# laiviet/ed-gated-gcn

Measured on AMD Instinct MI355X. Metric: gated_gcn_forward_edges_per_sec, higher is better.
Workload: dtype f32 (fp16 MFMA + block-scaled fp8 correction MFMA, fp32 accumulate)

## Files before the change

### ed-gated-gcn_amd/csrc/f16mx8_core.h

```cpp
#pragma once
#include "bf16x3_core.h"
#include "lab_hooks.h"

namespace ggcn {
namespace mx8 {

using namespace bx3;

typedef _Float16 f16x8 __attribute__((ext_vector_type(8)));
typedef int i32x8 __attribute__((ext_vector_type(8)));
typedef int i32x4 __attribute__((ext_vector_type(4)));

#ifndef GGCN_WH8_STORED
#define GGCN_WH8_STORED 0
#endif
constexpr int kWh8Bytes = GGCN_WH8_STORED ? 64 * 16 : 0;
constexpr int kOffWl8 = 2 * 1024, kOffWh8 = kOffWl8 + 64 * 16, kOffScales = kOffWh8 + kWh8Bytes;
constexpr int STAGE_PACK_BYTES = kOffScales + 64 * 4;
constexpr int XL_SHIFT = 11;
constexpr int SCALE_XL = 127 - XL_SHIFT, SCALE_XH = 127;

static __device__ unsigned int g_range_flag;
constexpr float kWindow = 448.0f;
constexpr float kHalfMax = 65504.0f;
__device__ __forceinline__ void range_verdict(float amax, float hb_scale = 0.0f, float hb_add = 0.0f, bool window = true)
{
    unsigned bits = 0u;
    if (window && amax > kWindow) bits |= 2u;
    if (amax >= kHalfMax) bits |= 1u;
    if (amax * hb_scale + hb_add >= kHalfMax) bits |= 4u;
    if (bits) atomicOr(&g_range_flag, bits);
}
#define GGCN_RANGE_FLAG_TU(fn)                                                                          \
    namespace {                                                                                         \
    __global__ void fn##_kernel(unsigned int *dst, int clear)                                           \
    {                                                                                                   \
        const unsigned int v = mx8::g_range_flag;                                                       \
        if (v) atomicOr(dst, v);                                                                        \
        if (clear) mx8::g_range_flag = 0u;                                                              \
    }                                                                                                   \
    }                                                                                                   \
    int fn(unsigned int *dst, int clear, hipStream_t st)                                                \
    {                                                                                                   \
        hipLaunchKernelGGL(fn##_kernel, dim3(1), dim3(1), 0, st, dst, clear);                           \
        return check_launch("ggcn_range_flag");                                                         \
    }
constexpr int PACK_TRAILER_BYTES = 16;
__device__ __forceinline__ float amax3(float x0, float x1, float m)
{
    float d;
    asm("v_max3_f32 %0, |%1|, |%2|, %3" : "=v"(d) : "v"(x0), "v"(x1), "v"(m));
    return d;
}

struct Split4 {
    uint32_t h01, h23;
    int l8, h8;
};
__device__ __forceinline__ int undef_vgpr() { int r; asm volatile("" : "=v"(r)); return r; }
__device__ __forceinline__ Split4 split4(float x0, float x1, float x2, float x3, float &amax)
{
    typedef _Float16 h2 __attribute__((ext_vector_type(2)));
    typedef float f2 __attribute__((ext_vector_type(2)));
    typedef short s2 __attribute__((ext_vector_type(2)));
    const h2 p0 = __builtin_convertvector(f2{x0, x1}, h2);
    const h2 p1 = __builtin_convertvector(f2{x2, x3}, h2);
    float r0, r1, r2, r3;
    asm("v_fma_mix_f32 %0, %1, -1.0, %2 op_sel_hi:[1,0,0]" : "=v"(r0) : "v"(p0), "v"(x0));
    asm("v_fma_mix_f32 %0, %1, -1.0, %2 op_sel:[1,0,0] op_sel_hi:[1,0,0]" : "=v"(r1) : "v"(p0), "v"(x1));
    asm("v_fma_mix_f32 %0, %1, -1.0, %2 op_sel_hi:[1,0,0]" : "=v"(r2) : "v"(p1), "v"(x2));
    asm("v_fma_mix_f32 %0, %1, -1.0, %2 op_sel:[1,0,0] op_sel_hi:[1,0,0]" : "=v"(r3) : "v"(p1), "v"(x3));
    constexpr float inv = 1.0f / (float)(1 << XL_SHIFT);
    s2 q = __builtin_bit_cast(s2, undef_vgpr());
    q = __builtin_amdgcn_cvt_scalef32_pk_fp8_f32(q, r0, r1, inv, false);
    q = __builtin_amdgcn_cvt_scalef32_pk_fp8_f32(q, r2, r3, inv, true);
    amax = amax3(x2, x3, amax3(x0, x1, amax));
    int h8 = __builtin_amdgcn_cvt_pk_fp8_f32(x0, x1, undef_vgpr(), false);
    h8 = __builtin_amdgcn_cvt_pk_fp8_f32(x2, x3, h8, true);
    Split4 o;
    o.h01 = __builtin_bit_cast(uint32_t, p0);
    o.h23 = __builtin_bit_cast(uint32_t, p1);
    o.l8 = __builtin_bit_cast(int, q);
    o.h8 = h8;
    return o;
}

__device__ __forceinline__ void set_cvt_saturate(bool on) { __builtin_amdgcn_s_setreg(1 | (23 << 6), on ? 1 : 0); }

__device__ __forceinline__ int q_lds_off(int row, int chunk)
{
    return row * ROWB + ((chunk ^ ((row >> 2) & 3) ^ (((row >> 1) & 1) << 1)) << 4);
}

#define GGCN_SB() __builtin_amdgcn_sched_barrier(0)
#define GGCN_ON(bit) constexpr (!((GGCN_LAB_OFF) & (bit)))

template <typename AT>
struct BufX {
    const AT *base;
    uint32_t bytes;
    uint32_t off[Geom<AT>::NP];
};
template <typename AT>
__device__ __forceinline__ BufX<AT> make_bufx(const AT *X, int64_t ldx, int64_t base_row, int64_t total_rows,
                                              const int (&rel)[Geom<AT>::NP], int tid)
{
    BufX<AT> b;
    const int64_t left = (total_rows - base_row) * ldx * (int64_t)sizeof(AT);
    b.base = X + base_row * ldx;
    b.bytes = (uint32_t)(left < 0x7fffffff ? left : 0x7fffffff);
#pragma unroll
    for (int i = 0; i < Geom<AT>::NP; ++i)
        b.off[i] = rel[i] < 0 ? 0x80000000u
                              : (uint32_t)(((int64_t)rel[i] * ldx + (tid % Geom<AT>::TPR) * Geom<AT>::EPT) * (int64_t)sizeof(AT));
    return b;
}
#ifndef GGCN_LAB_W2
#define GGCN_LAB_W2 0
#endif
template <typename AT, bool AVEC, bool KFULL, bool ZROWS, bool RBLK = false, bool BUF = false, int NB = 4, bool XS = false, int XP = 4, int SLOT0 = 0>
__device__ __forceinline__ void mainloop(const AT *const (&arow)[Geom<AT>::NP], const bool (&avalid)[Geom<AT>::NP],
                                         const char *__restrict__ wpack, int K, int stages_packed, int wm,
                                         int nt0, int n_tiles_total, char *lds, f32x16 (&acc)[4][RN], int rot = 0, int nblk = 4,
                                         float *amax_out = nullptr, const BufX<AT> *bufx = nullptr, float xscale = 1.0f, int pass0 = 0)
{
    static_assert(!BUF || (AVEC && KFULL && sizeof(AT) == 4), "buffer loads: whole 16-byte pieces of fp32 rows");
    static_assert(NB >= 1 && NB <= 4 && (NB == 4 || (sizeof(AT) == 4 && !RBLK)), "NB < 4: fp32 rows (pass i = block i), no run-time count");
    constexpr int NPL0 = Geom<AT>::NP < NB ? Geom<AT>::NP : NB;
    constexpr int NPL = NPL0 < XP ? NPL0 : XP;
    static_assert(XP == 4 || (sizeof(AT) == 4 && NB == 4 && !RBLK), "XP < 4: fp32 rows, whole tiles");
    static_assert(SLOT0 >= 0 && SLOT0 + XP <= 4, "the staging passes sit behind the stage's four row-block slots");
    using G = Geom<AT>;
    constexpr int EPT = G::EPT, NP = G::NP, NQ = EPT / 4;
    static_assert(BK == 32 && NP <= 4 && RN == 2, "the slot schedule below is written for BK = 32, <= 4 passes, RN = 2");
    const int tid = threadIdx.x & (kThreads - 1);
    const int lane = tid & 63;
    const int s_k = (tid % G::TPR) * EPT;

    set_cvt_saturate(true);
    float amax = 0.0f;

    constexpr int kRsrcFlags = 0x00020000;
    __amdgpu_buffer_rsrc_t xr, wr;
    if constexpr (BUF) {
        xr = __builtin_amdgcn_make_buffer_rsrc(const_cast<AT *>(bufx->base), 0, (int)bufx->bytes, kRsrcFlags);
        wr = __builtin_amdgcn_make_buffer_rsrc(const_cast<char *>(wpack), 0, 0x7fffffff, kRsrcFlags);
    }
    float ra[NP][EPT];
    auto load_a_pass = [&](int i, int k0) {
        const int gk = k0 + s_k;
        if constexpr (BUF) {
            const float4 t = __builtin_bit_cast(float4, __builtin_amdgcn_raw_buffer_load_b128(xr, bufx->off[i], k0 * (int)sizeof(AT), 0));
            ra[i][0] = t.x; ra[i][1] = t.y; ra[i][2] = t.z; ra[i][3] = t.w;
        } else if constexpr (AVEC) {
            load16<AT>(arow[i] + ((KFULL || gk < K) ? gk : 0), ra[i]);
        } else {
#pragma unroll
            for (int c = 0; c < EPT; ++c) ra[i][c] = elem_to_float(arow[i][(gk + c < K) ? gk + c : 0]);
        }
    };
    Split4 sp[NQ];
    auto split_pass = [&](int i, int k0) {
        const int gk = k0 + s_k;
#pragma unroll
        for (int q = 0; q < NQ; ++q) {
            float x[4];
#pragma unroll
            for (int c = 0; c < 4; ++c) {
                x[c] = ra[i][4 * q + c];
                if constexpr (!KFULL || ZROWS) {
                    bool in = true;
                    if constexpr (!KFULL) in = gk + 4 * q + c < K;
                    if constexpr (ZROWS && !BUF) in = in && avalid[i];
                    x[c] = in ? x[c] : 0.0f;
                }
                if constexpr (XS) x[c] *= xscale;
            }
            sp[q] = split4(x[0], x[1], x[2], x[3], amax);
        }
    };
    auto write_pass = [&](int buf, int i) {
        char *h_plane = lds + buf * (2 * BM * ROWB);
        char *q_plane = h_plane + BM * ROWB;
        const int row = stage_row<AT>(XP == 4 ? i : i + pass0);
#pragma unroll
        for (int q = 0; q < NQ; ++q) {
            const int kq = s_k + 4 * q;
            *reinterpret_cast<uint2 *>(h_plane + a_lds_off(row, kq >> 3) + (kq & 4) * 2) = make_uint2(sp[q].h01, sp[q].h23);
            const int g = kq >> 2, hh = (g >> 1) & 1, pos = (g & 1) + 2 * (g >> 2);
            *reinterpret_cast<uint32_t *>(q_plane + q_lds_off(row, hh) + 4 * pos) = (uint32_t)sp[q].l8;
            *reinterpret_cast<uint32_t *>(q_plane + q_lds_off(row, 2 + hh) + 4 * pos) = (uint32_t)sp[q].h8;
        }
    };

    const char *bbase[RN];
#pragma unroll
    for (int j = 0; j < RN; ++j) {
        const int ntc = nt0 + j < n_tiles_total ? nt0 + j : n_tiles_total - 1;
        bbase[j] = wpack + (int64_t)ntc * stages_packed * STAGE_PACK_BYTES + lane * 16;
    }
    uint32_t wtile[RN];
#pragma unroll
    for (int j = 0; j < RN; ++j) {
        const int ntc = nt0 + j < n_tiles_total ? nt0 + j : n_tiles_total - 1;
        wtile[j] = (uint32_t)ntc * (uint32_t)stages_packed * STAGE_PACK_BYTES;
    }
    const uint32_t lane16 = lane * 16, lane4 = lane * 4;
    auto load_bf = [&](int st, f16x8 (&b0)[RN], f16x8 (&b1)[RN]) {
        st = st < stages_packed ? st : stages_packed - 1;
#pragma unroll
        for (int j = 0; j < RN; ++j) {
            if constexpr (BUF) {
                const uint32_t so = wtile[j] + (uint32_t)st * STAGE_PACK_BYTES;
                b0[j] = __builtin_bit_cast(f16x8, __builtin_amdgcn_raw_buffer_load_b128(wr, lane16, so, 0));
                b1[j] = __builtin_bit_cast(f16x8, __builtin_amdgcn_raw_buffer_load_b128(wr, lane16, so + 1024, 0));
            } else {
                const char *p = bbase[j] + (int64_t)st * STAGE_PACK_BYTES;
                b0[j] = *reinterpret_cast<const f16x8 *>(p);
                b1[j] = *reinterpret_cast<const f16x8 *>(p + 1024);
            }
        }
    };
    auto load_bq = [&](int st, i32x4 (&b)[RN], int (&sc)[RN]) {
        st = st < stages_packed ? st : stages_packed - 1;
#pragma unroll
        for (int j = 0; j < RN; ++j) {
            if constexpr (BUF) {
                const uint32_t so = wtile[j] + (uint32_t)st * STAGE_PACK_BYTES;
                b[j] = __builtin_bit_cast(i32x4, __builtin_amdgcn_raw_buffer_load_b128(wr, lane16, so + kOffWl8, 0));
                sc[j] = __builtin_amdgcn_raw_buffer_load_b32(wr, lane4, so + kOffScales, 0);
            } else {
                const char *p = bbase[j] + (int64_t)st * STAGE_PACK_BYTES;
                b[j] = *reinterpret_cast<const i32x4 *>(p + kOffWl8);
                sc[j] = *reinterpret_cast<const int *>(p + kOffScales - lane * 12);
            }
        }
    };
    auto load_wh8 = [&](int st, i32x4 (&b)[RN]) {
        st = st < stages_packed ? st : stages_packed - 1;
#pragma unroll
        for (int j = 0; j < RN; ++j) {
            if constexpr (BUF) b[j] = __builtin_bit_cast(i32x4, __builtin_amdgcn_raw_buffer_load_b128(wr, lane16, wtile[j] + (uint32_t)st * STAGE_PACK_BYTES + kOffWh8, 0));
            else b[j] = *reinterpret_cast<const i32x4 *>(bbase[j] + (int64_t)st * STAGE_PACK_BYTES + kOffWh8);
        }
    };
    auto wh8_of = [&](const f16x8 &f0, const f16x8 &f1, int sc) -> i32x4 {
        typedef _Float16 h2 __attribute__((ext_vector_type(2)));
        typedef short s2 __attribute__((ext_vector_type(2)));
        const float inv = __builtin_bit_cast(float, (sc & 0xff00) << 15);
        i32x4 o;
#pragma unroll
        for (int d = 0; d < 4; ++d) {
            const f16x8 &f = d < 2 ? f0 : f1;
            const int e = (d & 1) * 4;
            s2 q = __builtin_bit_cast(s2, undef_vgpr());
            q = __builtin_amdgcn_cvt_scalef32_pk_fp8_f16(q, h2{f[e], f[e + 1]}, inv, false);
            q = __builtin_amdgcn_cvt_scalef32_pk_fp8_f16(q, h2{f[e + 2], f[e + 3]}, inv, true);
            o[d] = __builtin_bit_cast(int, q);
        }
        return o;
    };

    const int f_row = wm * 128 + (lane & 31);
    const int f_half = lane >> 5;
    const int scale_a = f_half ? SCALE_XH : SCALE_XL;
    auto read_h = [&](int buf, int i, f16x8 (&a)[2]) {
        const char *h_plane = lds + buf * (2 * BM * ROWB);
        const int row = f_row + i * 32;
        a[0] = *reinterpret_cast<const f16x8 *>(h_plane + a_lds_off(row, f_half));
        a[1] = *reinterpret_cast<const f16x8 *>(h_plane + a_lds_off(row, 2 + f_half));
    };
    auto read_q = [&](int buf, int i, i32x8 &a) {
        const char *q_plane = lds + buf * (2 * BM * ROWB) + BM * ROWB;
        const int row = f_row + i * 32;
        const i32x4 lo = *reinterpret_cast<const i32x4 *>(q_plane + q_lds_off(row, f_half));
        const i32x4 hi = *reinterpret_cast<const i32x4 *>(q_plane + q_lds_off(row, 2 + f_half));
        a = __builtin_shufflevector(lo, hi, 0, 1, 2, 3, 4, 5, 6, 7);
    };

#pragma unroll
    for (int i = 0; i < 4; ++i)
#pragma unroll
        for (int j = 0; j < RN; ++j)
#pragma unroll
            for (int r = 0; r < 16; ++r) acc[i][j][r] = 0.0f;

    constexpr bool W2 = (GGCN_LAB_W2) != 0;
    f16x8 bset0[W2 ? 2 : 1][RN], bset1[W2 ? 2 : 1][RN];
    f16x8 (&b0)[RN] = bset0[0], (&b1)[RN] = bset1[0];
    i32x4 bq[RN];
    i32x4 bw[RN];
    int sq[RN];
    const int stages = (K + BK - 1) / BK;

    auto kstage = [&](int n) {
        n = n < stages ? n : stages - 1;
        const int s = n + rot;
        return s >= stages ? s - stages : s;
    };
#pragma unroll
    for (int p = 0; p < NPL; ++p) load_a_pass(p, kstage(0) * BK);
    load_bf(kstage(0), b0, b1);
#pragma unroll
    for (int p = 0; p < NPL; ++p) {
        split_pass(p, kstage(0) * BK);
        write_pass(0, p);
    }
#pragma unroll
    for (int p = 0; p < NPL; ++p) load_a_pass(p, kstage(1) * BK);
    __syncthreads();

    f16x8 lab_h[2];
    i32x8 lab_q;
    i32x8 lab_bm[RN];
    if constexpr ((GGCN_LAB_OFF) != 0) {
        read_h(0, 0, lab_h);
        read_q(0, 0, lab_q);
        load_bq(kstage(0), bq, sq);
        if constexpr (GGCN_WH8_STORED) load_wh8(kstage(0), bw);
#pragma unroll
        for (int j = 0; j < RN; ++j) {
            const i32x4 w = GGCN_WH8_STORED ? bw[j] : wh8_of(b0[j], b1[j], sq[j]);
            lab_bm[j] = i32x8{w[0], w[1], w[2], w[3], bq[j][0], bq[j][1], bq[j][2], bq[j][3]};
        }
    }
    auto stage = [&](int st, auto bufc) {
        constexpr int buf = decltype(bufc)::value;
        const int k_next1 = kstage(st + 1) * BK;
        const int ka = kstage(st + 2) * BK;
        f16x8 ah[2][2];
        i32x8 aq[2];
        if GGCN_ON(8) read_h(buf, 0, ah[0]); else { ah[0][0] = lab_h[0]; ah[0][1] = lab_h[1]; }
        if GGCN_ON(16) { load_bq(kstage(st), bq, sq); if constexpr (GGCN_WH8_STORED) load_wh8(kstage(st), bw); }
        f16x8 (&b0)[RN] = bset0[W2 ? buf : 0], (&b1)[RN] = bset1[W2 ? buf : 0];
        if constexpr (W2) { if GGCN_ON(16) load_bf(kstage(st + 1), bset0[buf ^ 1], bset1[buf ^ 1]); }
        GGCN_SB();
#pragma unroll
        for (int i = 0; i < NB; ++i) {
            if GGCN_ON(8) {
                if (i < NB - 1) read_h(buf, i + 1, ah[(i + 1) & 1]);
                else read_q(buf, 0, aq[0]);
            } else {
                if (i < NB - 1) { ah[(i + 1) & 1][0] = lab_h[0]; ah[(i + 1) & 1][1] = lab_h[1]; }
                else aq[0] = lab_q;
            }
            GGCN_SB();
            if (!RBLK || i < nblk) acc[i][0] = __builtin_amdgcn_mfma_f32_32x32x16_f16(ah[i & 1][0], b0[0], acc[i][0], 0, 0, 0);
            GGCN_SB();
            if GGCN_ON(2) { if (i - SLOT0 >= 0 && i - SLOT0 < NP && i - SLOT0 < GGCN_LAB_XPASSES && i - SLOT0 < XP) split_pass(i - SLOT0, k_next1); }
            GGCN_SB();
            if (!RBLK || i < nblk) acc[i][1] = __builtin_amdgcn_mfma_f32_32x32x16_f16(ah[i & 1][0], b0[1], acc[i][1], 0, 0, 0);
            GGCN_SB();
            if GGCN_ON(4) { if (i - SLOT0 >= 0 && i - SLOT0 < NP && i - SLOT0 < GGCN_LAB_XPASSES && i - SLOT0 < XP) write_pass(buf ^ 1, i - SLOT0); }
            else { _Pragma("unroll") for (int q = 0; q < NQ; ++q) asm volatile("" :: "v"(sp[q].h01), "v"(sp[q].h23), "v"(sp[q].l8), "v"(sp[q].h8)); }
            GGCN_SB();
            if (!RBLK || i < nblk) acc[i][0] = __builtin_amdgcn_mfma_f32_32x32x16_f16(ah[i & 1][1], b1[0], acc[i][0], 0, 0, 0);
            GGCN_SB();
            if GGCN_ON(1) { if (i - SLOT0 >= 0 && i - SLOT0 < NP && i - SLOT0 < GGCN_LAB_XPASSES && i - SLOT0 < XP) load_a_pass(i - SLOT0, ka); }
            else { if (i < NP) { _Pragma("unroll") for (int c = 0; c < EPT; ++c) asm volatile("" : "+v"(ra[i][c])); } }
            GGCN_SB();
            if (!RBLK || i < nblk) acc[i][1] = __builtin_amdgcn_mfma_f32_32x32x16_f16(ah[i & 1][1], b1[1], acc[i][1], 0, 0, 0);
            GGCN_SB();
        }
        i32x8 bm[RN];
        auto make_bm = [&](int j) {
            if GGCN_ON(32) {
                i32x4 w;
                if constexpr (GGCN_WH8_STORED) w = bw[j];
                else w = wh8_of(b0[j], b1[j], sq[j]);
                bm[j] = i32x8{w[0], w[1], w[2], w[3], bq[j][0], bq[j][1], bq[j][2], bq[j][3]};
            } else {
                bm[j] = lab_bm[j];
            }
        };
        make_bm(0);
        if constexpr (!(GGCN_LAB_WH8)) make_bm(1);
        GGCN_SB();
#pragma unroll
        for (int i = 0; i < NB; ++i) {
            if GGCN_ON(8) { if (i < NB - 1) read_q(buf, i + 1, aq[(i + 1) & 1]); }
            else { if (i < NB - 1) aq[(i + 1) & 1] = lab_q; }
            GGCN_SB();
            if (!RBLK || i < nblk) acc[i][0] = __builtin_amdgcn_mfma_scale_f32_32x32x64_f8f6f4(aq[i & 1], bm[0], acc[i][0], GGCN_LAB_MXFMT, GGCN_LAB_MXFMT, 0, scale_a, 0, sq[0]);
            GGCN_SB();
            if constexpr (GGCN_LAB_WH8) { if (i == 0) make_bm(1); }
            if constexpr (!W2) { if GGCN_ON(16) { if (i == 0) load_bf(kstage(st + 1), b0, b1); } }
            GGCN_SB();
            if (!RBLK || i < nblk) acc[i][1] = __builtin_amdgcn_mfma_scale_f32_32x32x64_f8f6f4(aq[i & 1], bm[1], acc[i][1], GGCN_LAB_MXFMT, GGCN_LAB_MXFMT, 0, scale_a, 0, sq[1]);
            GGCN_SB();
        }
        if GGCN_ON(64) __syncthreads();
    };
    int st = 0;
    for (; st + 1 < stages; st += 2) {
        stage(st, std::integral_constant<int, 0>{});
        stage(st + 1, std::integral_constant<int, 1>{});
    }
    if (st < stages) stage(st, std::integral_constant<int, 0>{});
    set_cvt_saturate(false);
    if (amax_out) *amax_out = amax;
    else range_verdict(amax);
}
#undef GGCN_SB
#undef GGCN_ON

}
}
```

### ed-gated-gcn_amd/csrc/fused_block8.hip

```cpp
#include "fused_common.h"

#include <cstdlib>

namespace ggcn {
namespace {

constexpr int kB8Threads = 512;
constexpr int kB8Lds = kLdsBytes + 2 * kEpiLdsBytes;

__device__ __forceinline__ bool getenv_slot_same(const FusedArgs &a) { return (a.k_steps & 0x20000000) != 0; }

template <int BASE>
__device__ __forceinline__ float staged_mid_max(const char *lds, bool dma, int lane)
{
    if (dma) {
        const float4 m4 = *reinterpret_cast<const float4 *>(lds + EpiLds<BASE>::kBias + BN * 4 + lane * 16);
        float mm = fmaxf(fmaxf(fabsf(m4.x), fabsf(m4.y)), fmaxf(fabsf(m4.z), fabsf(m4.w)));
#pragma unroll
        for (int d = 32; d >= 1; d >>= 1) mm = fmaxf(mm, __shfl_xor(mm, d));
        return mm;
    }
    const float4 mm = *reinterpret_cast<const float4 *>(lds + EpiLds<BASE>::kMidMax);
    return fmaxf(fmaxf(mm.x, mm.y), fmaxf(mm.z, mm.w));
}

template <bool FULLT, bool VST>
__global__ __launch_bounds__(kB8Threads, 1) void block_fused8_kernel(const FusedArgs a)
{
    extern __shared__ __attribute__((aligned(16))) char lds[];
    const int B = a.B, T = a.T, K = a.K, F = a.F;
    int n_wgi, g_tile;
    if (a.n_parts == 2) {
        const int xcd = blockIdx.x & 7, qb = blockIdx.x >> 3;
        const int total = a.g_tiles * a.n_wg, per_xcd = (total + 7) >> 3;
        const int w = xcd * per_xcd + qb;
        if (qb >= per_xcd || w >= total) return;
        n_wgi = w / a.g_tiles;
        g_tile = w - n_wgi * a.g_tiles;
    } else {
        if (!tile_of_block(blockIdx.x, a.g_tiles, a.n_wg, g_tile, n_wgi)) return;
    }

    const int tid8 = threadIdx.x;
    const unsigned long long t_start = a.stamps ? __builtin_amdgcn_s_memrealtime() : 0;
    const int group = __builtin_amdgcn_readfirstlane(tid8 >> 8);
    const int tid = tid8 & 255;
    const int wave = __builtin_amdgcn_readfirstlane(tid >> 6);
    const LayerPart &lp = a.part[group];
    const int gt0 = g_tile * 4, g0 = gt0;
    const int n_tiles_total = (F + NT - 1) / NT;
    const int nt0 = n_wgi * (BN / NT) + wave * RN;

    constexpr int NP = Geom<float>::NP;
    const float *arow[NP];
    bool avalid[NP];
    int rel[NP];
#pragma unroll
    for (int i = 0; i < NP; ++i) {
        const int row = stage_row<float>(i < 2 ? i + 2 * group : 0);
        const int g = gt0 + (row >> 5), r = row & 31;
        avalid[i] = i < 2 && (g < B) && (FULLT || r < T);
        arow[i] = a.X;
        rel[i] = avalid[i] ? (row >> 5) * T + (row & 31) : -1;
    }
    const bool dma = (a.n_wg * BN == F) && (gt0 + 4 <= B) && a.ov_in == nullptr && a.ov_out == nullptr && (a.k_steps & 0x40000000) != 0;
    const int k_steps = a.k_steps & 0x1fffffff;
    if (dma) {
        if (group == 0) stage_epilogue_operands_dma<kLdsBytes>(a, lp, g0, n_wgi, lds, tid);
        else stage_epilogue_operands_dma<kLdsBytes + kEpiLdsBytes>(a, lp, g0, n_wgi, lds, tid);
    } else {
        if (group == 0) stage_epilogue_operands<kLdsBytes>(a, lp, g0, n_wgi, lds, tid);
        else stage_epilogue_operands<kLdsBytes + kEpiLdsBytes>(a, lp, g0, n_wgi, lds, tid);
    }

    f32x16 acc[4][RN];
    float amax;
    const int64_t pack_bytes = (int64_t)n_tiles_total * (k_steps / 2) * mx8::STAGE_PACK_BYTES;
    const float bw1 = *reinterpret_cast<const float *>(a.part[0].wpack + pack_bytes);
    const float bw12 = *reinterpret_cast<const float *>(a.part[1].wpack + pack_bytes);
    const unsigned long long t_loop0 = a.stamps ? __builtin_amdgcn_s_memrealtime() : 0;
    mx8::BufX<float> bx = mx8::make_bufx<float>(a.X, a.ldx, (int64_t)gt0 * T, (int64_t)B * T, rel, tid);
    if (group == 0 || getenv_slot_same(a))
        mx8::mainloop<float, true, true, !FULLT, false, true, 4, false, 2, 0>(arow, avalid, lp.wpack, K, k_steps / 2, 0, nt0, n_tiles_total, lds, acc, 0, 4,
                                                                               &amax, &bx, 1.0f, 2 * group);
    else
        mx8::mainloop<float, true, true, !FULLT, false, true, 4, false, 2, 2>(arow, avalid, lp.wpack, K, k_steps / 2, 0, nt0, n_tiles_total, lds, acc, 0, 4,
                                                                               &amax, &bx, 1.0f, 2 * group);
    unsigned long long t_loop1 = 0;
    if (a.stamps) { asm volatile("" :: "v"(acc[3][RN - 1][15])); t_loop1 = __builtin_amdgcn_s_memrealtime(); }
    mx8::range_verdict(amax, bw12, staged_mid_max<kLdsBytes + kEpiLdsBytes>(lds, dma, tid & 63), true);
    mx8::range_verdict(amax, bw1, 0.0f, false);
    if (group == 0) {
        epilogue<1, FULLT, VST, false, false, kLdsBytes>(a, lp, acc, g0, nt0, n_tiles_total, lds, tid);
    } else {
        if (lp.out) epilogue<1, FULLT, VST, true, true, kLdsBytes + kEpiLdsBytes>(a, lp, acc, g0, nt0, n_tiles_total, lds, tid);
        else epilogue<1, FULLT, VST, true, false, kLdsBytes + kEpiLdsBytes>(a, lp, acc, g0, nt0, n_tiles_total, lds, tid);
    }
    if (a.stamps && tid == 0) {
        unsigned long long *o = a.stamps + ((size_t)blockIdx.x * 2 + group) * 4;
        o[0] = t_start; o[1] = t_loop0; o[2] = t_loop1; o[3] = __builtin_amdgcn_s_memrealtime();
    }
}

}

int device_cu_count()
{
    static int cus = 0;
    if (cus == 0) {
        int dev = 0, n = 0;
        if (hipGetDevice(&dev) != hipSuccess || hipDeviceGetAttribute(&n, hipDeviceAttributeMultiprocessorCount, dev) != hipSuccess || n <= 0) n = 256;
        cus = n;
    }
    return cus;
}
bool block8_shape(int B, int T, int K, int F)
{
    if (B <= 0 || T > 32 || T <= 0 || F <= 0 || K <= 0 || F % BN != 0 || K % BK != 0) return false;
    const int64_t total = (int64_t)((B + 3) / 4) * (F / BN), cus = device_cu_count();
    return total >= 6 * cus || (total >= 3 * cus && total % cus == 0);
}
bool block8_takes(const float *X, int64_t ldx, const void *wpack1, const void *wpack12, int B, int T, int K, int F, const float *gate1,
                  const float *gate2, const float *bias1, const float *bias_mid, const float *bias2, const void *graph_ops,
                  const void *graph_ops2, const float *x_out, int64_t ld2)
{
    if (!block8_shape(B, T, K, F)) return false;
    if (ldx < K || !aligned16(wpack1) || !aligned16(wpack12) || (x_out && ld2 < F)) return false;
    if (!((ldx % 4 == 0) && aligned16(X) && (int64_t)ldx * 4 * 257 < ((int64_t)1 << 31))) return false;
    if (!graph_ops || !graph_ops2 || !gate1 || !gate2 || !bias_mid) return false;
    if (!(aligned16(gate1) && aligned16(gate2) && aligned16(bias1) && aligned16(bias2) && aligned16(bias_mid) && aligned16(graph_ops) &&
          aligned16(graph_ops2)))
        return false;
    if (x_out && !((ld2 % 4 == 0) && aligned16(x_out) && (int64_t)T * ld2 * 4 < ((int64_t)1 << 31))) return false;
    return true;
}

int lab_block_fused8(const float *X, int64_t ldx, const void *wpack1, const void *wpack12, const void *graph_ops, const void *graph_ops2,
                     const float *bias1, const float *bias_mid, const float *bias2, int B, int T, int K, int F, const float *gate1,
                     const float *gate2, float *x_out, int64_t ld2, float *x1, float *y1, float *pool_out, float *overlap_partial,
                     hipStream_t st, unsigned long long *stamps, int flags)
{
    const char *who = (flags & kBlock8Product) ? "ggcn_block_fused" : "ggcn_lab_block_fused8";
    if (!X || !wpack1 || !wpack12 || !graph_ops || !graph_ops2 || !gate1 || !gate2 || !x1 || !y1 || !bias_mid)
        return fail(GGCN_EINVAL, "%s: null pointer", who);
    if (B <= 0 || T <= 0 || T > 32 || K <= 0 || F <= 0) return fail(GGCN_EUNSUPPORTED, "%s: B=%d T=%d K=%d F=%d (graphs of <= 32 nodes)", who, B, T, K, F);
    if (ldx < K) return fail(GGCN_EINVAL, "%s: ldx < K", who);
    if (!aligned16(wpack1) || !aligned16(wpack12)) return fail(GGCN_EINVAL, "%s: wpack must be 16-byte aligned", who);
    if (x_out && ld2 < F) return fail(GGCN_EINVAL, "%s: leading dimension of the output too small", who);
    const bool avec = (K % 4 == 0) && (ldx % 4 == 0) && aligned16(X) && (int64_t)ldx * 4 * 257 < ((int64_t)1 << 31);
    if (!avec || K % BK != 0) return fail(GGCN_EUNSUPPORTED, "%s: fast shapes only (K %% 32 == 0, 16-byte aligned rows)", who);
    if (!x_out && !pool_out) return fail(GGCN_EINVAL, "%s: neither x nor its pool requested", who);
    FusedArgs a = {};
    a.X = X; a.ldx = ldx; a.graph_ops = static_cast<const char *>(graph_ops); a.graph_ops2 = static_cast<const char *>(graph_ops2);
    const bool rowmajor = (flags & kBlock8RowMajor) != 0;
    a.B = B; a.T = T; a.K = K; a.F = F; a.n_parts = rowmajor ? 3 : 2;
    a.part[0] = LayerPart{static_cast<const char *>(wpack1), bias1, nullptr, nullptr, nullptr, gate1, gate2, nullptr, x1, y1, overlap_partial, 0};
    a.part[1] = LayerPart{static_cast<const char *>(wpack12), bias2, bias_mid, nullptr, gate2, gate2, nullptr, x_out, pool_out, nullptr, nullptr, (int)ld2};
    a.stamps = stamps;
    a.k_steps = round_up(K, BK) / KSTEP;
    const bool al = (F % 4 == 0) && aligned16(gate1) && aligned16(gate2) && aligned16(bias1) && aligned16(bias2) && aligned16(bias_mid) &&
                    aligned16(graph_ops) && aligned16(graph_ops2) && !(flags & kBlock8NoDma);
    if (al) a.k_steps |= 0x40000000;
    if (flags & kBlock8SameSlots) a.k_steps |= 0x20000000;
    a.n_wg = (F + BN - 1) / BN;
    a.g_tiles = (B + 3) / 4;
    const bool vst = x_out && (F % 4 == 0) && (ld2 % 4 == 0) && aligned16(x_out) && (int64_t)T * ld2 * 4 < ((int64_t)1 << 31);
    if (x_out && !vst) return fail(GGCN_EUNSUPPORTED, "%s: x needs F %% 4 == 0 and 16-byte aligned rows", who);
    const bool fullt = (T == 32) && (B % 4 == 0);
    const int64_t total = (int64_t)a.g_tiles * a.n_wg;
    const int64_t grid = rowmajor ? grid_for(a.g_tiles, a.n_wg) : 8 * ((total + 7) / 8);
    if (grid > (int64_t)INT32_MAX) return fail(GGCN_EUNSUPPORTED, "%s: batch too large", who);
#define GGCN_L8(FT, VS)                                                                                                           \
    do {                                                                                                                          \
        auto kern = block_fused8_kernel<FT, VS>;                                                                                  \
        if (hipFuncSetAttribute(reinterpret_cast<const void *>(kern), hipFuncAttributeMaxDynamicSharedMemorySize, kB8Lds) != hipSuccess) \
            return fail(GGCN_ELAUNCH, "%s: cannot reserve %d bytes of LDS", who, kB8Lds);                                         \
        hipLaunchKernelGGL(kern, dim3((unsigned)grid), dim3(kB8Threads), kB8Lds, st, a);                                          \
    } while (0)
    if (fullt && vst) GGCN_L8(true, true);
    else if (fullt) GGCN_L8(true, false);
    else if (vst) GGCN_L8(false, true);
    else GGCN_L8(false, false);
#undef GGCN_L8
    return check_launch(who);
}

GGCN_RANGE_FLAG_TU(range_flag_block8)

}
```

### ed-gated-gcn_amd/csrc/fused_common.h

```cpp
#pragma once
#include "f16mx8_core.h"
#include "dropout_hash.h"
#include "lab_hooks.h"

namespace ggcn {

struct LayerPart {
    const char *wpack;
    const float *bias;
    const float *mid;
    const float *pre;
    const float *store_gate;
    const float *pool_gate_a;
    const float *pool_gate_b;
    float *out;
    float *pool_a, *pool_b;
    float *ov_partial;
    int ldo;
};

struct FusedArgs {
    const float *X;
    int64_t ldx;
    const uint32_t *rowmask;
// ... 161 lines not shown
}


template <int BASE>
struct EpiLds {
    static constexpr int kOps = BASE;
    static constexpr int kGate = kOps + 4 * kOps2Bytes;
    static constexpr int kBias = kGate + 3 * 4 * BN * 4;
    static constexpr int kMidMax = kBias + 2 * BN * 4;
    static constexpr int kEnd = kMidMax + 16;
};
constexpr int kEpiLdsBytes = EpiLds<0>::kEnd;
static_assert(WM == 1, "one wavefront row: the workgroup's 4 graphs are every wavefront's 4 graphs");

template <int BASE, bool GIVEN = false>
__device__ __forceinline__ void stage_epilogue_operands(const FusedArgs &a, const LayerPart &lp, int g0, int n_wgi, char *lds, int tid,
                                                        const char *given = nullptr)
{
    constexpr int kEpiOps = EpiLds<BASE>::kOps, kEpiGate = EpiLds<BASE>::kGate, kEpiBias = EpiLds<BASE>::kBias;
    const int B = a.B, F = a.F;
    constexpr int kPieceIts = (4 * kOps2Bytes / 16 + kThreads - 1) / kThreads;
    uint4 piece[kPieceIts];
    const bool second = GIVEN || lp.mid != nullptr;
    const int blk_bytes = second ? kOps2Bytes : kOpsBytes;
    const char *ops_src = GIVEN ? given : second ? a.graph_ops2 : a.graph_ops;
    const int n_pieces = 4 * blk_bytes / 16;
#pragma unroll
    for (int it = 0; it < kPieceIts; ++it) {
        const int idx = tid + it * kThreads;
        const int idc = idx < n_pieces ? idx : 0;
        const int gi = (idc * 16) / blk_bytes;
        const int64_t off = (int64_t)g0 * blk_bytes + (g0 + gi < B ? idc * 16 : idc * 16 - gi * blk_bytes);
        piece[it] = *reinterpret_cast<const uint4 *>(ops_src + off);
    }
    const int col = n_wgi * BN + tid;
    const bool cok = col < F;
    const float *dummy = a.X;
    const float *gp[3] = {lp.store_gate, lp.pool_gate_a, lp.pool_gate_b};
    float gv[3][4];
#pragma unroll
    for (int k = 0; k < 3; ++k)
#pragma unroll
        for (int i = 0; i < 4; ++i) {
            const bool ok = gp[k] && cok && g0 + i < B;
            const float v = (gp[k] ? gp[k] : dummy)[ok ? (int64_t)(g0 + i) * F + col : 0];
            gv[k][i] = ok ? v : 1.0f;
        }
    const float vbias = (lp.bias ? lp.bias : dummy)[lp.bias && cok ? col : 0];
    const float vmidb = (lp.mid ? lp.mid : dummy)[lp.mid && cok ? col : 0];
#pragma unroll
    for (int it = 0; it < kPieceIts; ++it) {
        const int idx = tid + it * kThreads;
        if (idx < n_pieces) *reinterpret_cast<uint4 *>(lds + kEpiOps + idx * 16) = piece[it];
    }
    float *gl = reinterpret_cast<float *>(lds + kEpiGate);
#pragma unroll
    for (int k = 0; k < 3; ++k)
#pragma unroll
        for (int i = 0; i < 4; ++i) gl[(k * 4 + i) * BN + tid] = gv[k][i];
    float *bl = reinterpret_cast<float *>(lds + kEpiBias);
    bl[tid] = lp.bias && cok ? vbias : 0.0f;
    bl[BN + tid] = lp.mid && cok ? vmidb : 0.0f;
    float mm = lp.mid && cok ? fabsf(vmidb) : 0.0f;
#pragma unroll
    for (int d = 32; d >= 1; d >>= 1) mm = fmaxf(mm, __shfl_xor(mm, d));
    if ((tid & 63) == 0) reinterpret_cast<float *>(lds + EpiLds<BASE>::kMidMax)[tid >> 6] = mm;
}

template <int BASE>
__device__ __forceinline__ void fused_range_verdict(float amax, const char *wpack, int64_t pack_bytes, const char *lds, bool window)
{
    const float bw = *reinterpret_cast<const float *>(wpack + pack_bytes);
    const float4 mm = *reinterpret_cast<const float4 *>(lds + EpiLds<BASE>::kMidMax);
    mx8::range_verdict(amax, bw, fmaxf(fmaxf(mm.x, mm.y), fmaxf(mm.z, mm.w)), window);
}

template <int BASE, bool GIVEN = false>
__device__ __forceinline__ void stage_epilogue_operands_dma(const FusedArgs &a, const LayerPart &lp, int g0, int n_wgi, char *lds, int tid,
                                                            const char *given = nullptr)
{
    constexpr int kEpiOps = EpiLds<BASE>::kOps, kEpiGate = EpiLds<BASE>::kGate, kEpiBias = EpiLds<BASE>::kBias;
    const int lane = tid & 63, wave = __builtin_amdgcn_readfirstlane(tid >> 6);
    const int F = a.F;
    const bool second = GIVEN || lp.mid != nullptr;
    const int total = 4 * (second ? kOps2Bytes : kOpsBytes);
    const char *src = (GIVEN ? given : second ? a.graph_ops2 : a.graph_ops) + (int64_t)g0 * (second ? kOps2Bytes : kOpsBytes);
    for (int piece = wave; piece * 1024 < total; piece += 4)
        if (piece * 1024 + lane * 16 < total)
            __builtin_amdgcn_global_load_lds((const __attribute__((address_space(1))) void *)(src + piece * 1024 + lane * 16),
                                             (__attribute__((address_space(3))) void *)(lds + kEpiOps + piece * 1024), 16, 0, 0);
    const float *gp[3] = {lp.store_gate, lp.pool_gate_a, lp.pool_gate_b};
    float *gl = reinterpret_cast<float *>(lds + kEpiGate);
#pragma unroll
    for (int k = 0; k < 3; ++k) {
        if (gp[k]) {
            __builtin_amdgcn_global_load_lds((const __attribute__((address_space(1))) void *)(gp[k] + (int64_t)(g0 + wave) * F + n_wgi * BN + lane * 4),
                                             (__attribute__((address_space(3))) void *)(lds + kEpiGate + ((k * 4 + wave) * BN) * 4), 16, 0, 0);
        } else {
#pragma unroll
            for (int i = 0; i < 4; ++i) gl[(k * 4 + i) * BN + tid] = 1.0f;
        }
    }
    float *bl = reinterpret_cast<float *>(lds + kEpiBias);
    if (lp.bias) {
        if (wave == 0) __builtin_amdgcn_global_load_lds((const __attribute__((address_space(1))) void *)(lp.bias + n_wgi * BN + lane * 4),
                                                        (__attribute__((address_space(3))) void *)(lds + kEpiBias), 16, 0, 0);
    } else bl[tid] = 0.0f;
    if (lp.mid) {
        if (wave == 1) __builtin_amdgcn_global_load_lds((const __attribute__((address_space(1))) void *)(lp.mid + n_wgi * BN + lane * 4),
                                                        (__attribute__((address_space(3))) void *)(lds + kEpiBias + BN * 4), 16, 0, 0);
    } else bl[BN + tid] = 0.0f;
}
template <int BASE>
__device__ __forceinline__ void dma_range_verdict(float amax, const char *wpack, int64_t pack_bytes, const char *lds, int lane)
{
    const float4 m4 = *reinterpret_cast<const float4 *>(lds + EpiLds<BASE>::kBias + BN * 4 + lane * 16);
    float mm = fmaxf(fmaxf(fabsf(m4.x), fabsf(m4.y)), fmaxf(fabsf(m4.z), fabsf(m4.w)));
#pragma unroll
    for (int d = 32; d >= 1; d >>= 1) mm = fmaxf(mm, __shfl_xor(mm, d));
    const float bw = *reinterpret_cast<const float *>(wpack + pack_bytes);
    mx8::range_verdict(amax, bw, mm, true);
}

__device__ __forceinline__ float vmax_raw(float x, float y) { float d; asm("v_max_f32 %0, %1, %2" : "=v"(d) : "v"(x), "v"(y)); return d; }
__device__ __forceinline__ float vmin_raw(float x, float y) { float d; asm("v_min_f32 %0, %1, %2" : "=v"(d) : "v"(x), "v"(y)); return d; }

__device__ __forceinline__ void meet_halves(float &vmax, float &vmin)
{
    const auto r = __builtin_amdgcn_permlane32_swap(__float_as_uint(vmax), __float_as_uint(vmin), false, false);
    const float a = __uint_as_float(r[0]), b = __uint_as_float(r[1]);
    const float m = vmax_raw(a, b), n = vmin_raw(a, b);
    const auto q = __builtin_amdgcn_permlane32_swap(__float_as_uint(n), __float_as_uint(a), false, false);
    vmax = m;
    vmin = __uint_as_float(q[1]);
}

__device__ __forceinline__ float wave_sum_to_lane0(float v)
{
    v += __uint_as_float(__builtin_amdgcn_update_dpp(0, __float_as_uint(v), 0xB1, 0xF, 0xF, true));
    v += __uint_as_float(__builtin_amdgcn_update_dpp(0, __float_as_uint(v), 0x4E, 0xF, 0xF, true));
    v += __uint_as_float(__builtin_amdgcn_update_dpp(0, __float_as_uint(v), 0x141, 0xF, 0xF, true));
    v += __uint_as_float(__builtin_amdgcn_update_dpp(0, __float_as_uint(v), 0x140, 0xF, 0xF, true));
    const float r1 = __uint_as_float(__builtin_amdgcn_readlane(__float_as_uint(v), 16));
    const float r2 = __uint_as_float(__builtin_amdgcn_readlane(__float_as_uint(v), 32));
    const float r3 = __uint_as_float(__builtin_amdgcn_readlane(__float_as_uint(v), 48));
    return (v + r1) + (r2 + r3);
}

__device__ __forceinline__ __amdgpu_buffer_rsrc_t out_rsrc(void *p)
{
    return __builtin_amdgcn_make_buffer_rsrc(p, 0, 0x7fffffff, 0x00020000);
}

template <int SCH, bool FULLT, bool VST, bool MID, bool OUT, int BASE = kLdsBytes, bool DROP = false>
__device__ __forceinline__ void epilogue(const FusedArgs &a, const LayerPart &lp, f32x16 (&acc)[4][RN], int g0, int nt0,
                                         int n_tiles_total, char *lds, int tid)
{
    constexpr int kEpiOps = EpiLds<BASE>::kOps, kEpiGate = EpiLds<BASE>::kGate, kEpiBias = EpiLds<BASE>::kBias;
    using P = AggPlane<SCH>;
    typedef typename P::frag frag;
    const int B = a.B, T = a.T, F = a.F;
    float *__restrict__ out = lp.out, *__restrict__ pool_a = lp.pool_a, *__restrict__ pool_b = lp.pool_b;
    float *__restrict__ ov_partial = lp.ov_partial;
    const int ldo = lp.ldo;
    const int lane = tid & 63;
    const int wave = __builtin_amdgcn_readfirstlane(tid >> 6);
    const int c = lane & 31, h = lane >> 5;

    const char *ops_lds = lds + kEpiOps;
    const float *gate_lds = reinterpret_cast<const float *>(lds + kEpiGate);
    const float *bias_lds = reinterpret_cast<const float *>(lds + kEpiBias);
    const int wn = wave % WN;
    float vb[RN], vmid[RN];
    bool col_ok[RN];
#pragma unroll
    for (int j = 0; j < RN; ++j) {
        col_ok[j] = (nt0 + j) * NT + c < F;
        vb[j] = bias_lds[wn * (RN * NT) + j * NT + c];
        vmid[j] = bias_lds[BN + wn * (RN * NT) + j * NT + c];
    }
    const int lane_off = 4 * h * ldo + c;
    float *stage_lds = reinterpret_cast<float *>(lds) + wave * (32 * 64);
    constexpr bool vst = VST && OUT;
    constexpr bool direct_store = !VST && OUT;

#pragma unroll
    for (int i = 0; i < 4; ++i) {
        const int g = g0 + i;
        if (!FULLT && g >= B) break;
        constexpr int kBlk = MID ? kOps2Bytes : kOpsBytes;
        constexpr int kRowOff = MID ? 4096 : 2048;
        frag afv[2], afl[2];
#pragma unroll
        for (int s = 0; s < 2; ++s) {
            const uint4 raw = *reinterpret_cast<const uint4 *>(ops_lds + i * kBlk + s * 1024 + lane * 16);
            union { frag v; uint32_t w[4]; } u;
            if constexpr (MID) {
                u.w[0] = raw.x; u.w[1] = raw.y; u.w[2] = raw.z; u.w[3] = raw.w;
                afv[s] = u.v;
                const uint4 rl = *reinterpret_cast<const uint4 *>(ops_lds + i * kBlk + 2048 + s * 1024 + lane * 16);
                u.w[0] = rl.x; u.w[1] = rl.y; u.w[2] = rl.z; u.w[3] = rl.w;
                afl[s] = u.v;
            } else {
                u.w[0] = raw.x & P::kOne; u.w[1] = raw.y & P::kOne;
                u.w[2] = raw.z & P::kOne; u.w[3] = raw.w & P::kOne;
                afv[s] = u.v;
            }
        }
        float4 rv[4];
#pragma unroll
        for (int q = 0; q < 4; ++q) rv[q] = *reinterpret_cast<const float4 *>(ops_lds + i * kBlk + kRowOff + h * 64 + q * 16);
        float vsg[RN], vga[RN], vgb[RN];
#pragma unroll
        for (int j = 0; j < RN; ++j) {
            const int at = i * BN + wn * (RN * NT) + j * NT + c;
            vsg[j] = gate_lds[at];
            vga[j] = gate_lds[4 * BN + at];
            vgb[j] = gate_lds[8 * BN + at];
        }
        bool tile_ok[RN];
#pragma unroll
        for (int j = 0; j < RN; ++j) tile_ok[j] = nt0 + j < n_tiles_total;

        f32x16 y[RN];
#pragma unroll
        for (int j = 0; j < RN; ++j) {
            frag hf[2][2];
            P::split(acc[i][j], hf);
#pragma unroll
            for (int r = 0; r < 16; ++r) y[j][r] = 0.0f;
            if constexpr (MID) {
#pragma unroll
                for (int s = 0; s < 2; ++s) y[j] = P::mma(afl[s], hf[0][s], y[j]);
#pragma unroll
                for (int s = 0; s < 2; ++s) y[j] = P::mma(afv[s], hf[1][s], y[j]);
#pragma unroll
                for (int s = 0; s < 2; ++s) y[j] = P::mma(afv[s], hf[0][s], y[j]);
            } else {
#pragma unroll
                for (int p = 1; p >= 0; --p)
#pragma unroll
                    for (int s = 0; s < 2; ++s) { if constexpr (!((GGCN_LAB_EPI) & 2)) y[j] = P::mma(afv[s], hf[p][s], y[j]); else y[j][s] += (float)hf[p][s][0]; }
            }
        }
        float rinv[16];
#pragma unroll
        for (int q = 0; q < 4; ++q) {
            rinv[4 * q] = rv[q].x; rinv[4 * q + 1] = rv[q].y; rinv[4 * q + 2] = rv[q].z; rinv[4 * q + 3] = rv[q].w;
        }
        float dot = 0.0f;
#pragma unroll
        for (int j = 0; j < RN; ++j) {
            if (!tile_ok[j]) break;
            const int gn = (nt0 + j) * NT + c;
            float vmax = -INFINITY, vmin = INFINITY, pmax_a = -INFINITY, pmax_b = -INFINITY;
            float *tile = OUT ? out + ((int64_t)g * T) * ldo + (nt0 + j) * NT : nullptr;
            const float sg = vsg[j];
            const float bj = vb[j];
            const uint32_t didx0 = DROP ? (uint32_t)(((int64_t)g * T + 4 * h) * F + gn) : 0u;
#pragma unroll
            for (int r = 0; r < 16; ++r) {
                const int row0 = (r & 3) + 8 * (r >> 2);
                const float v = MID ? fmaf(y[j][r], kM2InvScale, fmaf(rinv[r], vmid[j], bj)) : y[j][r] * rinv[r] + bj;
                float vs = v * sg;
                if constexpr (DROP) {
                    const uint32_t hh = drop_hash(didx0 + (uint32_t)(row0 * F), a.drop.seed_lo, a.drop.seed_hi);
                    vs *= drop_keep(hh, a.drop.sel[0], a.drop.thr, a.drop.scale);
                    if (FULLT || row0 + 4 * h < T) {
                        pmax_a = fmaxf(pmax_a, v * vga[j] * drop_keep(hh, a.drop.sel[1], a.drop.thr, a.drop.scale));
                        pmax_b = fmaxf(pmax_b, v * vgb[j] * drop_keep(hh, a.drop.sel[2], a.drop.thr, a.drop.scale));
                    }
                }
                if constexpr (vst) {
                    stage_lds[(row0 + 4 * h) * 64 + ((32 * j + c) ^ (32 * h))] = vs;
                }
                if (FULLT || row0 + 4 * h < T) {
                    if (direct_store && col_ok[j]) tile[lane_off + row0 * ldo] = vs;
                    if constexpr (!DROP) {
                        vmax = fmaxf(vmax, v);
                        vmin = fminf(vmin, v);
                    }
                }
            }
            float pa, pb;
            if constexpr (DROP) {
                pa = fmaxf(pmax_a, upper_half_to_lower(pmax_a));
                pb = fmaxf(pmax_b, upper_half_to_lower(pmax_b));
            } else {
                meet_halves(vmax, vmin);
                const float ga = vga[j], gb = vgb[j];
                pa = ga * (ga >= 0.0f ? vmax : vmin);
                pb = gb * (gb >= 0.0f ? vmax : vmin);
            }
            if (h == 0 && col_ok[j]) {
                if (pool_a) __builtin_amdgcn_raw_buffer_store_b32(__float_as_uint(pa), out_rsrc(pool_a + (int64_t)g * F), 4 * gn, 0, 0);
                if (pool_b) __builtin_amdgcn_raw_buffer_store_b32(__float_as_uint(pb), out_rsrc(pool_b + (int64_t)g * F), 4 * gn, 0, 0);
                dot = fmaf(pa, pb, dot);
            }
        }
        if (ov_partial && nt0 < n_tiles_total) {
            const float tot = wave_sum_to_lane0(dot);
            if (lane == 0) ov_partial[(int64_t)g * ((F + 63) / 64) + (nt0 >> 1)] = tot;
        }
        if constexpr (vst) {
            __builtin_amdgcn_fence(__ATOMIC_RELEASE, "wavefront");
            __builtin_amdgcn_wave_barrier();
            const int colq = (lane & 15) * 4;
            const int gcol = nt0 * NT + colq;
            const __amdgpu_buffer_rsrc_t orsrc = out_rsrc(out + ((int64_t)g * T) * ldo);
            const int voff = ((lane >> 4) * ldo + gcol) * 4;
#pragma unroll
            for (int it = 0; it < 8; ++it) {
                const int row = 4 * it + (lane >> 4);
                const float4 v4 = *reinterpret_cast<const float4 *>(&stage_lds[row * 64 + (colq ^ (32 * ((row >> 2) & 1)))]);
                typedef uint32_t u32x4 __attribute__((ext_vector_type(4)));
                if ((FULLT || row < T) && gcol < F && !((GGCN_LAB_EPI) & 1))
                    __builtin_amdgcn_raw_buffer_store_b128(__builtin_bit_cast(u32x4, v4), orsrc, voff, 4 * it * ldo * 4, (GGCN_LAB_NT_STORE) ? 2 : 0);
            }
            __builtin_amdgcn_fence(__ATOMIC_ACQUIRE, "wavefront");
            __builtin_amdgcn_wave_barrier();
        }
        if (i == 0) GGCN_TRACE(7);
    }
}


}
}
```

Baseline: 804.4 million.

## Let only one workgroup per row tile track range and stage full mid row

Adds a TRACK template flag so that only the first workgroup of each row group (n_wgi == 0) computes the amax of the split inputs and issues the range verdict. That workgroup stages the whole mid-bias row into extra dynamic LDS to take its max. The other workgroups skip the amax3 ops and the verdict. The second group's epilogue also drops the pool_b gate, its stores and the overlap dot partial. Dynamic LDS now grows with F (capped at 16384 columns), which may reduce occupancy for large F, and correctness relies on the speaking workgroup covering the same rows.

```diff
diff --git a/ed-gated-gcn_amd/csrc/f16mx8_core.h b/ed-gated-gcn_amd/csrc/f16mx8_core.h
--- a/ed-gated-gcn_amd/csrc/f16mx8_core.h
+++ b/ed-gated-gcn_amd/csrc/f16mx8_core.h
@@ -58,6 +58,7 @@
     int l8, h8;
 };
 __device__ __forceinline__ int undef_vgpr() { int r; asm volatile("" : "=v"(r)); return r; }
+template <bool TRACK = true>
 __device__ __forceinline__ Split4 split4(float x0, float x1, float x2, float x3, float &amax)
 {
     typedef _Float16 h2 __attribute__((ext_vector_type(2)));
@@ -74,7 +75,7 @@
     s2 q = __builtin_bit_cast(s2, undef_vgpr());
     q = __builtin_amdgcn_cvt_scalef32_pk_fp8_f32(q, r0, r1, inv, false);
     q = __builtin_amdgcn_cvt_scalef32_pk_fp8_f32(q, r2, r3, inv, true);
-    amax = amax3(x2, x3, amax3(x0, x1, amax));
+    if constexpr (TRACK) amax = amax3(x2, x3, amax3(x0, x1, amax));
     int h8 = __builtin_amdgcn_cvt_pk_fp8_f32(x0, x1, undef_vgpr(), false);
     h8 = __builtin_amdgcn_cvt_pk_fp8_f32(x2, x3, h8, true);
     Split4 o;
@@ -118,7 +119,8 @@
 #ifndef GGCN_LAB_W2
 #define GGCN_LAB_W2 0
 #endif
-template <typename AT, bool AVEC, bool KFULL, bool ZROWS, bool RBLK = false, bool BUF = false, int NB = 4, bool XS = false, int XP = 4, int SLOT0 = 0>
+template <typename AT, bool AVEC, bool KFULL, bool ZROWS, bool RBLK = false, bool BUF = false, int NB = 4, bool XS = false, int XP = 4, int SLOT0 = 0,
+          bool TRACK = true>
 __device__ __forceinline__ void mainloop(const AT *const (&arow)[Geom<AT>::NP], const bool (&avalid)[Geom<AT>::NP],
                                          const char *__restrict__ wpack, int K, int stages_packed, int wm,
                                          int nt0, int n_tiles_total, char *lds, f32x16 (&acc)[4][RN], int rot = 0, int nblk = 4,
@@ -176,7 +178,7 @@
                 }
                 if constexpr (XS) x[c] *= xscale;
             }
-            sp[q] = split4(x[0], x[1], x[2], x[3], amax);
+            sp[q] = split4<TRACK>(x[0], x[1], x[2], x[3], amax);
         }
     };
     auto write_pass = [&](int buf, int i) {
@@ -398,8 +400,9 @@
     }
     if (st < stages) stage(st, std::integral_constant<int, 0>{});
     set_cvt_saturate(false);
+    static_assert(TRACK || XP < 4, "TRACK = false: only where another workgroup splits the same rows and speaks for them");
     if (amax_out) *amax_out = amax;
-    else range_verdict(amax);
+    else if constexpr (TRACK) range_verdict(amax);
 }
 #undef GGCN_SB
 #undef GGCN_ON
diff --git a/ed-gated-gcn_amd/csrc/fused_block8.hip b/ed-gated-gcn_amd/csrc/fused_block8.hip
--- a/ed-gated-gcn_amd/csrc/fused_block8.hip
+++ b/ed-gated-gcn_amd/csrc/fused_block8.hip
@@ -7,21 +7,35 @@
 
 constexpr int kB8Threads = 512;
 constexpr int kB8Lds = kLdsBytes + 2 * kEpiLdsBytes;
+constexpr int kB8MaxF = 16384;
+static_assert(kB8Lds % 16 == 0 && kB8Lds + kB8MaxF * 4 <= 160 * 1024, "the mid row behind the epilogue operands, 16-byte pieces");
+__host__ __device__ constexpr int b8_lds_bytes(int F) { return kB8Lds + (F + BN - 1) / BN * BN * 4; }
 
 __device__ __forceinline__ bool getenv_slot_same(const FusedArgs &a) { return (a.k_steps & 0x20000000) != 0; }
 
-template <int BASE>
-__device__ __forceinline__ float staged_mid_max(const char *lds, bool dma, int lane)
-{
-    if (dma) {
-        const float4 m4 = *reinterpret_cast<const float4 *>(lds + EpiLds<BASE>::kBias + BN * 4 + lane * 16);
-        float mm = fmaxf(fmaxf(fabsf(m4.x), fabsf(m4.y)), fmaxf(fabsf(m4.z), fabsf(m4.w)));
+__device__ __forceinline__ void stage_mid_row(const float *mid, int F, bool aligned, char *row, int tid)
+{
+    const int lane = tid & 63, wave = __builtin_amdgcn_readfirstlane(tid >> 6);
+    if (aligned) {
+        for (int piece = wave; piece * BN < F; piece += 4)
+            if (piece * BN + lane * 4 < F)
+                __builtin_amdgcn_global_load_lds((const __attribute__((address_space(1))) void *)(mid + piece * BN + lane * 4),
+                                                 (__attribute__((address_space(3))) void *)(row + piece * (BN * 4)), 16, 0, 0);
+    } else {
+        float *r = reinterpret_cast<float *>(row);
+        for (int idx = tid; idx < ((F + 3) & ~3); idx += 256) r[idx] = idx < F ? mid[idx] : 0.0f;
+    }
+}
+__device__ __forceinline__ float staged_mid_row_max(const char *row, int F, int lane)
+{
+    float mm = 0.0f;
+    for (int c = lane * 4; c < F; c += 256) {
+        const float4 m4 = *reinterpret_cast<const float4 *>(row + c * 4);
+        mm = fmaxf(mm, fmaxf(fmaxf(fabsf(m4.x), fabsf(m4.y)), fmaxf(fabsf(m4.z), fabsf(m4.w))));
+    }
 #pragma unroll
-        for (int d = 32; d >= 1; d >>= 1) mm = fmaxf(mm, __shfl_xor(mm, d));
-        return mm;
-    }
-    const float4 mm = *reinterpret_cast<const float4 *>(lds + EpiLds<BASE>::kMidMax);
-    return fmaxf(fmaxf(mm.x, mm.y), fmaxf(mm.z, mm.w));
+    for (int d = 32; d >= 1; d >>= 1) mm = fmaxf(mm, __shfl_xor(mm, d));
+    return mm;
 }
 
 template <bool FULLT, bool VST>
@@ -72,34 +86,43 @@
         if (group == 0) stage_epilogue_operands<kLdsBytes>(a, lp, g0, n_wgi, lds, tid);
         else stage_epilogue_operands<kLdsBytes + kEpiLdsBytes>(a, lp, g0, n_wgi, lds, tid);
     }
-
-    f32x16 acc[4][RN];
-    float amax;
+    const bool speaks = n_wgi == 0;
+    if (speaks && group == 1) stage_mid_row(a.part[1].mid, F, (a.k_steps & 0x40000000) != 0, lds + kB8Lds, tid);
+
     const int64_t pack_bytes = (int64_t)n_tiles_total * (k_steps / 2) * mx8::STAGE_PACK_BYTES;
     const float bw1 = *reinterpret_cast<const float *>(a.part[0].wpack + pack_bytes);
     const float bw12 = *reinterpret_cast<const float *>(a.part[1].wpack + pack_bytes);
     const unsigned long long t_loop0 = a.stamps ? __builtin_amdgcn_s_memrealtime() : 0;
     mx8::BufX<float> bx = mx8::make_bufx<float>(a.X, a.ldx, (int64_t)gt0 * T, (int64_t)B * T, rel, tid);
-    if (group == 0 || getenv_slot_same(a))
-        mx8::mainloop<float, true, true, !FULLT, false, true, 4, false, 2, 0>(arow, avalid, lp.wpack, K, k_steps / 2, 0, nt0, n_tiles_total, lds, acc, 0, 4,
-                                                                               &amax, &bx, 1.0f, 2 * group);
-    else
-        mx8::mainloop<float, true, true, !FULLT, false, true, 4, false, 2, 2>(arow, avalid, lp.wpack, K, k_steps / 2, 0, nt0, n_tiles_total, lds, acc, 0, 4,
-                                                                               &amax, &bx, 1.0f, 2 * group);
-    unsigned long long t_loop1 = 0;
-    if (a.stamps) { asm volatile("" :: "v"(acc[3][RN - 1][15])); t_loop1 = __builtin_amdgcn_s_memrealtime(); }
-    mx8::range_verdict(amax, bw12, staged_mid_max<kLdsBytes + kEpiLdsBytes>(lds, dma, tid & 63), true);
-    mx8::range_verdict(amax, bw1, 0.0f, false);
-    if (group == 0) {
-        epilogue<1, FULLT, VST, false, false, kLdsBytes>(a, lp, acc, g0, nt0, n_tiles_total, lds, tid);
-    } else {
-        if (lp.out) epilogue<1, FULLT, VST, true, true, kLdsBytes + kEpiLdsBytes>(a, lp, acc, g0, nt0, n_tiles_total, lds, tid);
-        else epilogue<1, FULLT, VST, true, false, kLdsBytes + kEpiLdsBytes>(a, lp, acc, g0, nt0, n_tiles_total, lds, tid);
-    }
-    if (a.stamps && tid == 0) {
-        unsigned long long *o = a.stamps + ((size_t)blockIdx.x * 2 + group) * 4;
-        o[0] = t_start; o[1] = t_loop0; o[2] = t_loop1; o[3] = __builtin_amdgcn_s_memrealtime();
-    }
+    auto rest = [&](auto track) {
+        constexpr bool TRACK = decltype(track)::value;
+        f32x16 acc[4][RN];
+        float amax;
+        if (group == 0 || getenv_slot_same(a))
+            mx8::mainloop<float, true, true, !FULLT, false, true, 4, false, 2, 0, TRACK>(arow, avalid, lp.wpack, K, k_steps / 2, 0, nt0, n_tiles_total,
+                                                                                         lds, acc, 0, 4, &amax, &bx, 1.0f, 2 * group);
+        else
+            mx8::mainloop<float, true, true, !FULLT, false, true, 4, false, 2, 2, TRACK>(arow, avalid, lp.wpack, K, k_steps / 2, 0, nt0, n_tiles_total,
+                                                                                         lds, acc, 0, 4, &amax, &bx, 1.0f, 2 * group);
+        unsigned long long t_loop1 = 0;
+        if (a.stamps) { asm volatile("" :: "v"(acc[3][RN - 1][15])); t_loop1 = __builtin_amdgcn_s_memrealtime(); }
+        if constexpr (TRACK) {
+            mx8::range_verdict(amax, bw12, staged_mid_row_max(lds + kB8Lds, F, tid & 63), true);
+            mx8::range_verdict(amax, bw1, 0.0f, false);
+        }
+        if (group == 0) {
+            epilogue<1, FULLT, VST, false, false, kLdsBytes>(a, lp, acc, g0, nt0, n_tiles_total, lds, tid);
+        } else {
+            if (lp.out) epilogue<1, FULLT, VST, true, true, kLdsBytes + kEpiLdsBytes, false, false>(a, lp, acc, g0, nt0, n_tiles_total, lds, tid);
+            else epilogue<1, FULLT, VST, true, false, kLdsBytes + kEpiLdsBytes, false, false>(a, lp, acc, g0, nt0, n_tiles_total, lds, tid);
+        }
+        if (a.stamps && tid == 0) {
+            unsigned long long *o = a.stamps + ((size_t)blockIdx.x * 2 + group) * 4;
+            o[0] = t_start; o[1] = t_loop0; o[2] = t_loop1; o[3] = __builtin_amdgcn_s_memrealtime();
+        }
+    };
+    if (speaks) rest(std::true_type{});
+    else rest(std::false_type{});
 }
 
 }
@@ -116,7 +139,7 @@
 }
 bool block8_shape(int B, int T, int K, int F)
 {
-    if (B <= 0 || T > 32 || T <= 0 || F <= 0 || K <= 0 || F % BN != 0 || K % BK != 0) return false;
+    if (B <= 0 || T > 32 || T <= 0 || F <= 0 || F > kB8MaxF || K <= 0 || F % BN != 0 || K % BK != 0) return false;
     const int64_t total = (int64_t)((B + 3) / 4) * (F / BN), cus = device_cu_count();
     return total >= 6 * cus || (total >= 3 * cus && total % cus == 0);
 }
@@ -143,7 +166,8 @@
     const char *who = (flags & kBlock8Product) ? "ggcn_block_fused" : "ggcn_lab_block_fused8";
     if (!X || !wpack1 || !wpack12 || !graph_ops || !graph_ops2 || !gate1 || !gate2 || !x1 || !y1 || !bias_mid)
         return fail(GGCN_EINVAL, "%s: null pointer", who);
-    if (B <= 0 || T <= 0 || T > 32 || K <= 0 || F <= 0) return fail(GGCN_EUNSUPPORTED, "%s: B=%d T=%d K=%d F=%d (graphs of <= 32 nodes)", who, B, T, K, F);
+    if (B <= 0 || T <= 0 || T > 32 || K <= 0 || F <= 0 || F > kB8MaxF)
+        return fail(GGCN_EUNSUPPORTED, "%s: B=%d T=%d K=%d F=%d (graphs of <= 32 nodes, <= %d columns)", who, B, T, K, F, kB8MaxF);
     if (ldx < K) return fail(GGCN_EINVAL, "%s: ldx < K", who);
     if (!aligned16(wpack1) || !aligned16(wpack12)) return fail(GGCN_EINVAL, "%s: wpack must be 16-byte aligned", who);
     if (x_out && ld2 < F) return fail(GGCN_EINVAL, "%s: leading dimension of the output too small", who);
@@ -170,12 +194,13 @@
     const int64_t total = (int64_t)a.g_tiles * a.n_wg;
     const int64_t grid = rowmajor ? grid_for(a.g_tiles, a.n_wg) : 8 * ((total + 7) / 8);
     if (grid > (int64_t)INT32_MAX) return fail(GGCN_EUNSUPPORTED, "%s: batch too large", who);
+    const int lds_bytes = b8_lds_bytes(F);
 #define GGCN_L8(FT, VS)                                                                                                           \
     do {                                                                                                                          \
         auto kern = block_fused8_kernel<FT, VS>;                                                                                  \
-        if (hipFuncSetAttribute(reinterpret_cast<const void *>(kern), hipFuncAttributeMaxDynamicSharedMemorySize, kB8Lds) != hipSuccess) \
-            return fail(GGCN_ELAUNCH, "%s: cannot reserve %d bytes of LDS", who, kB8Lds);                                         \
-        hipLaunchKernelGGL(kern, dim3((unsigned)grid), dim3(kB8Threads), kB8Lds, st, a);                                          \
+        if (hipFuncSetAttribute(reinterpret_cast<const void *>(kern), hipFuncAttributeMaxDynamicSharedMemorySize, lds_bytes) != hipSuccess) \
+            return fail(GGCN_ELAUNCH, "%s: cannot reserve %d bytes of LDS", who, lds_bytes);                                      \
+        hipLaunchKernelGGL(kern, dim3((unsigned)grid), dim3(kB8Threads), lds_bytes, st, a);                                       \
     } while (0)
     if (fullt && vst) GGCN_L8(true, true);
     else if (fullt) GGCN_L8(true, false);
diff --git a/ed-gated-gcn_amd/csrc/fused_common.h b/ed-gated-gcn_amd/csrc/fused_common.h
--- a/ed-gated-gcn_amd/csrc/fused_common.h
+++ b/ed-gated-gcn_amd/csrc/fused_common.h
@@ -337,10 +337,11 @@
     return __builtin_amdgcn_make_buffer_rsrc(p, 0, 0x7fffffff, 0x00020000);
 }
 
-template <int SCH, bool FULLT, bool VST, bool MID, bool OUT, int BASE = kLdsBytes, bool DROP = false>
+template <int SCH, bool FULLT, bool VST, bool MID, bool OUT, int BASE = kLdsBytes, bool DROP = false, bool PB = true>
 __device__ __forceinline__ void epilogue(const FusedArgs &a, const LayerPart &lp, f32x16 (&acc)[4][RN], int g0, int nt0,
                                          int n_tiles_total, char *lds, int tid)
 {
+    static_assert(PB || !DROP, "the dropout form pools through both gates");
     constexpr int kEpiOps = EpiLds<BASE>::kOps, kEpiGate = EpiLds<BASE>::kGate, kEpiBias = EpiLds<BASE>::kBias;
     using P = AggPlane<SCH>;
     typedef typename P::frag frag;
@@ -401,7 +402,7 @@
             const int at = i * BN + wn * (RN * NT) + j * NT + c;
             vsg[j] = gate_lds[at];
             vga[j] = gate_lds[4 * BN + at];
-            vgb[j] = gate_lds[8 * BN + at];
+            vgb[j] = PB ? gate_lds[8 * BN + at] : 0.0f;
         }
         bool tile_ok[RN];
 #pragma unroll
@@ -475,15 +476,15 @@
                 meet_halves(vmax, vmin);
                 const float ga = vga[j], gb = vgb[j];
                 pa = ga * (ga >= 0.0f ? vmax : vmin);
-                pb = gb * (gb >= 0.0f ? vmax : vmin);
+                pb = PB ? gb * (gb >= 0.0f ? vmax : vmin) : 0.0f;
             }
             if (h == 0 && col_ok[j]) {
                 if (pool_a) __builtin_amdgcn_raw_buffer_store_b32(__float_as_uint(pa), out_rsrc(pool_a + (int64_t)g * F), 4 * gn, 0, 0);
-                if (pool_b) __builtin_amdgcn_raw_buffer_store_b32(__float_as_uint(pb), out_rsrc(pool_b + (int64_t)g * F), 4 * gn, 0, 0);
-                dot = fmaf(pa, pb, dot);
+                if (PB && pool_b) __builtin_amdgcn_raw_buffer_store_b32(__float_as_uint(pb), out_rsrc(pool_b + (int64_t)g * F), 4 * gn, 0, 0);
+                if constexpr (PB) dot = fmaf(pa, pb, dot);
             }
         }
-        if (ov_partial && nt0 < n_tiles_total) {
+        if (PB && ov_partial && nt0 < n_tiles_total) {
             const float tot = wave_sum_to_lane0(dot);
             if (lane == 0) ov_partial[(int64_t)g * ((F + 63) / 64) + (nt0 >> 1)] = tot;
         }
```

Result: no change. 808.5 million, median of 6 (+0.5%).
